# f90/Wave-U-Net

Measured on AMD Instinct MI355X. Metric: waveform samples/sec fwd+bwd, M1 12-level Wave-U-Net @1/2/4/8 GPU, higher is better.
Workload: dtype f32

## Files before the change

include/wun.h:

```cpp
#ifndef WUN_H
#define WUN_H

#include <stdint.h>

#ifdef __cplusplus
extern "C" {
#endif

typedef enum wun_status {
    WUN_OK = 0,
    WUN_ERR_INVALID = -1,
    WUN_ERR_UNSUPPORTED = -2,
    WUN_ERR_HIP = -3,
    WUN_ERR_NOMEM = -4
} wun_status;

typedef struct wun_config {
    int32_t num_layers;
    int32_t num_initial_filters;
    int32_t filter_size;
    int32_t merge_filter_size;
    int32_t input_filter_size;
    int32_t output_filter_size;
    int32_t upsampling;
// ... 512 lines not shown
#define WUN_OP_FIRST_CONV        7
#define WUN_PATH_NONE          0
#define WUN_PATH_SCALAR        1
#define WUN_PATH_VEC4          2
#define WUN_PATH_VEC8_BF16     3
#define WUN_PATH_ONE_STAGE     4
#define WUN_PATH_TWO_STAGE     5
#define WUN_PATH_GENERIC       6
#define WUN_PATH_FOUR_POSITION 7
#define WUN_PATH_NOT_FUSED     8
#define WUN_PATH_FUSED         9
#define WUN_PATH_FIRST_CONV    10
#define WUN_OP_WGRAD             8
#define WUN_PATH_WGRAD_DIRECT  11
#define WUN_PATH_WGRAD_SPLIT   12
int wun_op_last_path(int op);

int64_t wun_op_conv1d_bf16_scratch(int cin, int cout, int k);
int wun_op_conv1d_bf16(const float* x, const float* w, const float* bias, float* y, float* scratch,
                       int batch, int cin, int cout, int k, int t_in, int t_out, int stride, int pad_left,
                       int lrelu, void* stream);

int64_t wun_op_conv1d_dgrad_bf16_scratch(int cin, int cout, int k);
int wun_op_conv1d_dgrad_bf16(const float* dz, const float* w, float* dx, float* scratch, int batch, int cin,
                             int cout, int k, int t_in, int t_out, int stride, int pad_left, void* stream);

#define WUN_BF16_VARIANT_BASE 1000

typedef struct wun_op_conv_bf16_desc {
    int32_t mode, B, C0, C1, N, N0, K, Tin, Tout, shift;
// ... 48 lines not shown
```

wave-u-net_amd/_lib.py:

```python
import ctypes as C
import os

_HERE = os.path.dirname(os.path.abspath(__file__))
LIB_PATH = os.path.join(_HERE, os.environ.get("WUN_LIB", "libwun.so"))


class WunConfig(C.Structure):
    _fields_ = [(n, C.c_int32) for n in (
        "num_layers", "num_initial_filters", "filter_size", "merge_filter_size",
        "input_filter_size", "output_filter_size", "upsampling", "output_type", "context",
        "num_sources", "num_channels", "output_activation", "compute_dtype", "exclusive_streams")]


class WunPlanInfo(C.Structure):
    _fields_ = [("batch", C.c_int64), ("input_frames", C.c_int64), ("output_frames", C.c_int64),
                ("num_params", C.c_int64), ("arena_floats", C.c_int64),
                ("workspace_floats", C.c_int64), ("num_tensors", C.c_int64),
                ("num_outputs", C.c_int64), ("fwd_flops", C.c_double), ("bwd_flops", C.c_double),
                ("fwd_flops_dense", C.c_double), ("fwd_flops_unique", C.c_double),
                ("bwd_flops_unique", C.c_double), ("compute_dtype_effective", C.c_int64)]


class WunActivationInfo(C.Structure):
    _fields_ = [(n, C.c_int64) for n in ("offset", "batch_stride", "pitch", "channels", "frames", "t0", "tstep", "elem_bytes")]
# ... 58 lines not shown


class WunOpWgradDesc(C.Structure):
    _fields_ = ([(n, C.c_int32) for n in ("family", "B", "C0", "C1", "N", "K", "x0_pitch", "x1_pitch", "rows_bf16", "nparts")] +
                [(n, C.c_int32 * 2) for n in ("loader", "x0_off", "x1_off", "Tin", "shift", "Tq", "dz_pitch", "nsplit")] +
                [(n, C.c_int32) for n in ("accumulate", "force_mtw", "force_nw", "planes", "zss", "et")] +
                [("plane_off", C.c_int32 * 4)])


WGRAD_LDS, WGRAD_WIN, WGRAD_BF16, WGRAD_NARROW = range(4)
BF16_VARIANT_BASE = 1000

(OP_UPSAMPLE, OP_UPSAMPLE_BACKWARD, OP_INTERP_GRAD, OP_HEAD_FORWARD, OP_HEAD_DFEAT, OP_CONV_EPILOGUE, OP_BTC_TO_NCW) = range(7)
OP_FIRST_CONV = 7
OP_WGRAD = 8
(PATH_NONE, PATH_SCALAR, PATH_VEC4, PATH_VEC8_BF16, PATH_ONE_STAGE, PATH_TWO_STAGE, PATH_GENERIC, PATH_FOUR_POSITION,
 PATH_NOT_FUSED, PATH_FUSED, PATH_FIRST_CONV, PATH_WGRAD_DIRECT, PATH_WGRAD_SPLIT) = range(13)

BLEND_NO_RISE, BLEND_NO_FALL = 1, 2
SNIPPET_SWAP, SNIPPET_NEGATE = 1, 2
SPEED_RATES, SPEED_MAX_RATIO = 8, 64
STRETCH_JOBS = 64
SNIPPET_ROWS = 24

SPEC_TT_Z, SPEC_TT_MEAN, SPEC_TT_VAR, SPEC_TT_ACT, SPEC_TT_DROPOUT = range(5)

_P = C.c_void_p
_SIGS = {
    "wun_get_padding": (C.c_int, [C.POINTER(WunConfig), C.c_int64, C.POINTER(C.c_int64),
                                  C.POINTER(C.c_int64)]),
# ... 326 lines not shown
```

wave-u-net_amd/csrc/wun_internal.h:

```cpp
#pragma once
#include <hip/hip_runtime.h>
#include <stdint.h>
#include <initializer_list>
#include <string>

namespace wun {

enum { LOADER_DIRECT = 0, LOADER_DEINT = 1 };

enum WunEarlyWindow { EW_DEFAULT, EW_OFF, EW_DEEP, EW_ALL };
enum WunEventScope { EV_DEFAULT, EV_SYSTEM, EV_DEVICE };
enum WunSidePrio { PRIO_DEFAULT, PRIO_LOW, PRIO_HIGH, PRIO_NORMAL };
struct WunSwitches {
    bool no_dedup = false;
    WunEarlyWindow early_window = EW_DEFAULT;
    bool odd_fuse_set = false;
    int odd_fuse_min = 64;
    bool no_odd_align = false;
    bool no_fuse_ups = false;
    bool bf16_head_serial = false;
    bool single_stream = false;
    WunSidePrio side_prio = PRIO_DEFAULT;
    WunEventScope event_scope = EV_DEFAULT;
    bool no_win = false;
// ... 74 lines not shown
    int KW;
    int loader;
    const float* dz; long long dzbs; int dzpitch; int N; int Tq;
    float* out;
    int direct;
    int split_base;
    int nsplit; int units_per_split; int nQT; int B;
    int ablate;
    int force_mtw, force_nw;
    int bf16;
    int win;
    int sbf;
    int accum;
};

struct WgradGeom { int MTW, NW, nMG, nNG, TK, XP, ZP, nChMax, ONESP, XW4; size_t lds; };
WgradGeom wgrad_geom(const WgradArgs& a);
bool wgrad_win_supported(const WgradArgs& a);
long long wgrad_win_partial_floats(const WgradArgs& a, const WunSwitches& sw);
int wgrad_win_units(const WgradArgs& a, const WunSwitches& sw);
int wgrad_win_tiles(const WgradArgs& a, const WunSwitches& sw);
hipError_t launch_wgrad_win(const WgradArgs& a, hipStream_t s, const WunSwitches& sw);
hipError_t launch_wgrad_win_reduce(const WgradArgs& a, const float* partial, int nsplit, float* out_w, float* out_b,
                                   hipStream_t s, const WunSwitches& sw);
struct WgradBfGeom { int MTW, NW, NCB, nCB, nMG, nNG, TK, XW4, XROWS, ZPe; size_t lds; };
bool wgrad_bf16_supported(const WgradArgs& a);
WgradBfGeom wgrad_bf16_geom(const WgradArgs& a);
hipError_t launch_wgrad_bf16(const WgradArgs& a, hipStream_t s);
hipError_t launch_wgrad_bf16_reduce(const WgradArgs& a, const float* partial, int nsplit, float* out_w, float* out_b,
                                    hipStream_t s);

struct NarrowWgradArgs {
// ... 189 lines not shown
```

wave-u-net_amd/csrc/wun_kernels.hip:

```cpp
#include "wun_device.h"

#include <cstdio>
#include <cstdlib>
#include <map>
#include <mutex>
#include <string>
#include <algorithm>
#include <vector>

namespace wun {

__device__ __forceinline__ f32x4 mfma16(float a, float b, f32x4 c) {
    return __builtin_amdgcn_mfma_f32_16x16x4f32(a, b, c, 0, 0, 0);
}

__host__ __device__ static inline int fit_pitch(int width, int mod32) {
    return width + (((mod32 - (width % 32)) % 32) + 32) % 32;
}

struct ProfSlot { std::string name; std::string tag; double flops; double bytes; hipEvent_t e0, e1, c0, c1; };
static std::vector<ProfSlot> g_prof;
static bool g_prof_on = false;
static bool g_prof_detail = false;
static std::mutex g_prof_mu;
// ... 1234 lines not shown
        WUN_CV(24, 6, 2, 4, 1, 8) WUN_CV(25, 6, 3, 4, 1, 8)
        WUN_CV4(26, 4, 3, 4, 1, 4) WUN_CV4(27, 2, 3, 4, 1, 4) WUN_CV4(28, 3, 3, 4, 1, 4) WUN_CV4(29, 2, 2, 4, 1, 4)
        WUN_CV4(30, 3, 2, 4, 1, 4) WUN_CV4(31, 4, 5, 4, 1, 4) WUN_CV4(32, 3, 5, 4, 1, 4) WUN_CV4(33, 2, 5, 4, 1, 4)
#define WUN_CF(i, MT, NW, WT, WN, CK) case i: return conv_launch_t<MT, NW, WT, WN, CK, true, true>(a, v, part, part_cap, s, sw);
        WUN_CF(34, 1, 2, 4, 1, 8) WUN_CF(35, 1, 3, 4, 1, 8) WUN_CF(36, 2, 2, 4, 1, 8) WUN_CF(37, 2, 3, 4, 1, 8)
        WUN_CF(38, 2, 3, 2, 2, 8) WUN_CF(39, 4, 3, 2, 2, 8) WUN_CF(40, 2, 2, 2, 2, 8) WUN_CF(41, 4, 2, 2, 2, 8)
#undef WUN_CF
        default: return hipErrorInvalidValue;
    }
#undef WUN_CV
#undef WUN_CV4
}

#define WUN_WG_XIT 8

template <int MTW, int NW, bool ACC = false>
__global__ __launch_bounds__(256, 2) void wgrad_mfma_kernel(WgradArgs a, int nMG, int nNG, int TK,
                                                         int XP, int ZP, int nChMax, int ONESP,
                                                         int XW4) {
    extern __shared__ __attribute__((aligned(16))) float lds[];
    constexpr int MG = 4 * MTW * 16;
    constexpr int NG = NW * 16;
    constexpr int ZIT = (NG * 32 + 255) / 256;
    const bool deint = (a.loader == LOADER_DEINT);
    const int planes = deint ? 2 : 1;
    float* Xs = lds + ONESP;
    float* Zs = Xs + nChMax * planes * XP;

    const int tid = threadIdx.x;
    const int lane = tid & 63;
    const int li = lane & 15, lg = lane >> 4;
    const int wave = __builtin_amdgcn_readfirstlane(tid >> 6);
    int bid = xcd_contiguous_block((int)blockIdx.x, (int)gridDim.x);
    const int ng = bid % nNG; bid /= nNG;
    const int mg = bid % nMG;
    const int split = bid / nMG;

    const int Ctot = a.C0 + a.C1;
    const int Mtot = Ctot * a.KW;
    const int rlo = mg * MG;
    const int cLo = rlo / a.KW;
    int cHi = (rlo + MG - 1) / a.KW;
    if (cHi > Ctot - 1) cHi = Ctot - 1;
    const int nCh = cHi - cLo + 1;

    const int delta0 = ((a.off0 - a.shift) % 4 + 4) % 4;
    const int delta1 = ((a.off1 - a.shift) % 4 + 4) % 4;

    int rowoff[MTW];
    int nact = 0;
#pragma unroll
    for (int mt = 0; mt < MTW; ++mt) {
        const int rt = rlo + (wave * MTW + mt) * 16;
        if (rt <= Mtot) nact = mt + 1;
        const int r = rt + li;
        int off = 0;
        if (r < Mtot) {
            const int c = r / a.KW, k = r - c * a.KW;
            const int kd = k + (c < a.C0 ? delta0 : delta1);
            off = ONESP + (c - cLo) * planes * XP + (deint ? ((kd & 1) * XP + (kd >> 1)) : kd);
        }
        rowoff[mt] = off;
    }
    for (int i = tid; i < ONESP; i += 256) lds[i] = 1.f;

    f32x4 acc[MTW][NW];
#pragma unroll
    for (int m = 0; m < MTW; ++m)
#pragma unroll
        for (int n = 0; n < NW; ++n) acc[m][n] = (f32x4){0.f, 0.f, 0.f, 0.f};

    f32x4 xreg[WUN_WG_XIT];
    f32x4 zreg[ZIT];
    const int TK4 = TK >> 2;
    const float inv_xw4 = 1.0f / (float)XW4, inv_tk4 = 1.0f / (float)TK4;

    int xpk[WUN_WG_XIT];
    int zpk[ZIT];
#pragma unroll
    for (int i = 0; i < WUN_WG_XIT; ++i) {
        const int f = tid + i * 256;
        const int row = (int)(((float)f + 0.5f) * inv_xw4);
        const int c4 = f - row * XW4;
        const bool rok = row < nCh;
        const int ldsoff = deint ? (row * 2) * XP + 2 * c4 : row * XP + 4 * c4;
        xpk[i] = rok ? (int)(0x80000000u | ((unsigned)row << 23) | ((unsigned)c4 << 16) | (unsigned)ldsoff)
                     : (int)((unsigned)c4 << 16);
    }
#pragma unroll
    for (int i = 0; i < ZIT; ++i) {
        const int f = tid + i * 256;
        const int row = (int)(((float)f + 0.5f) * inv_tk4);
        const int c4 = f - row * TK4;
        zpk[i] = row < NG ? (int)(0x80000000u | ((unsigned)row << 23) | ((unsigned)c4 << 16) | (unsigned)(row * ZP + 4 * c4))
                          : (int)((unsigned)c4 << 16);
    }

    auto load_unit = [&](int u) {
        const int b = u / a.nQT, qt = u - b * a.nQT;
        const int q0 = qt * TK;
        const int tb = (deint ? 2 * q0 : q0) - a.shift;
        const float* base0 = a.src0 + (long long)b * a.bs0;
        const float* base1 = (a.C1 > 0) ? a.src1 + (long long)b * a.bs1 : base0;
        const int e00 = (tb + a.off0) & ~3, e01 = (tb + a.off1) & ~3;
#pragma unroll
        for (int i = 0; i < WUN_WG_XIT; ++i) {
            int pk = xpk[i];
            asm volatile("" : "+v"(pk));
            int c = cLo + ((pk >> 23) & 255);
            c = c < Ctot ? c : Ctot - 1;
            const bool s1 = c >= a.C0;
            const int xro = s1 ? (c - a.C0) * a.pitch1 : c * a.pitch0;
            int e = (s1 ? e01 : e00) + (((pk >> 16) & 127) << 2);
            const int emax = (s1 ? a.pitch1 : a.pitch0) - 4;
            e = e < 0 ? 0 : (e > emax ? emax : e);
            xreg[i] = *reinterpret_cast<const f32x4*>((s1 ? base1 : base0) + xro + e);
        }
        const float* zb = a.dz + (long long)b * a.dzbs;
        const int qmax = a.dzpitch - 4;
#pragma unroll
        for (int i = 0; i < ZIT; ++i) {
            int pk = zpk[i];
            asm volatile("" : "+v"(pk));
            const int nn = ng * NG + ((pk >> 23) & 255);
            const int zro = (pk < 0 && nn < a.N ? nn : 0) * a.dzpitch;
            int q = q0 + (((pk >> 16) & 127) << 2);
            q = q > qmax ? qmax : q;
            zreg[i] = *reinterpret_cast<const f32x4*>(zb + zro + q);
        }
    };
    auto store_unit = [&](int u) {
        const int b = u / a.nQT, qt = u - b * a.nQT;
        const int q0 = qt * TK;
        const int tb = (deint ? 2 * q0 : q0) - a.shift;
        int nq = a.Tq - q0; if (nq > TK) nq = TK;
        const int span = 4 * XW4;
        const int t00 = ((tb + a.off0) & ~3) - a.off0, t01 = ((tb + a.off1) & ~3) - a.off1;
        const bool xedge = t00 < 0 || t00 + span > a.Tin || (a.C1 > 0 && (t01 < 0 || t01 + span > a.Tin));
#pragma unroll
        for (int i = 0; i < WUN_WG_XIT; ++i) {
            int pk = xpk[i];
            asm volatile("" : "+v"(pk));
            if (pk < 0) {
                f32x4 v = xreg[i];
                if (xedge) {
                    const bool s1 = cLo + ((pk >> 23) & 255) >= a.C0;
                    const int t0 = (s1 ? t01 : t00) + (((pk >> 16) & 127) << 2);
#pragma unroll
                    for (int k = 0; k < 4; ++k)
                        if (t0 + k < 0 || t0 + k >= a.Tin) v[k] = 0.f;
                }
                float* dstp = Xs + (pk & 0xFFFF);
                if (!deint) {
                    *reinterpret_cast<f32x4*>(dstp) = v;
                } else {
                    *reinterpret_cast<float2*>(dstp) = make_float2(v[0], v[2]);
                    *reinterpret_cast<float2*>(dstp + XP) = make_float2(v[1], v[3]);
                }
            }
        }
        const bool zedge = nq < TK;
#pragma unroll
        for (int i = 0; i < ZIT; ++i) {
            int pk = zpk[i];
            asm volatile("" : "+v"(pk));
            if (pk < 0) {
                f32x4 v = zreg[i];
                if (zedge) {
                    const int c4x = ((pk >> 16) & 127) << 2;
#pragma unroll
                    for (int k = 0; k < 4; ++k)
                        if (c4x + k >= nq) v[k] = 0.f;
                }
                float* p = Zs + (pk & 0xFFFF);
                *reinterpret_cast<float2*>(p) = make_float2(v[0], v[1]);
                *reinterpret_cast<float2*>(p + 2) = make_float2(v[2], v[3]);
            }
        }
        (void)b;
    };

    const int nunits = a.B * a.nQT;
    const int u0 = split * a.units_per_split;
    int u1 = u0 + a.units_per_split;
    if (u1 > nunits) u1 = nunits;
    constexpr bool wb_noload = false, wb_nostore = false, wb_nomfma = false, wb_noepi = false;
    if (u0 < u1 && !wb_noload) load_unit(u0);
    for (int u = u0; u < u1; ++u) {
        const int qt = u % a.nQT;
        int nq = a.Tq - qt * TK; if (nq > TK) nq = TK;
        const int nsteps = (nq + 3) >> 2;
        __syncthreads();
        if (!wb_nostore) store_unit(u);
        __syncthreads();
        if (u + 1 < u1 && !wb_noload) load_unit(u + 1);
        if (!wb_nomfma) {
            auto run_unit = [&](auto full_tag) {
                constexpr bool FULL = decltype(full_tag)::value;
                float a0[MTW], b0[NW], a1[MTW], b1[NW];
                auto ldop = [&](int st, float (&av)[MTW], float (&bv)[NW]) {
#pragma unroll
                    for (int mt = 0; mt < MTW; ++mt) av[mt] = lds[rowoff[mt] + 4 * st + lg];
#pragma unroll
                    for (int n = 0; n < NW; ++n) bv[n] = Zs[(n * 16 + li) * ZP + 4 * st + lg];
                };
// ... 51 lines not shown
            for (int n = 0; n < NW; ++n) tile[(mt * NW + n) * 64] = acc[mt][n];
        return;
    }
    float* outp = a.out;
#pragma unroll
    for (int mt = 0; mt < MTW; ++mt) {
        if (mt >= nact) continue;
#pragma unroll
        for (int n = 0; n < NW; ++n) {
            const int col = ng * NG + n * 16 + li;
            if (col >= a.N) continue;
#pragma unroll
            for (int r4 = 0; r4 < 4; ++r4) {
                const int r = rlo + (wave * MTW + mt) * 16 + lg * 4 + r4;
                if (r < Mtot) {
                    const int c = r / a.KW, k = r - c * a.KW;
                    grad_st<ACC>(&outp[((long long)k * Ctot + c) * a.N + col], acc[mt][n][r4]);
                } else if (r == Mtot) {
                    grad_st<ACC>(&outp[(long long)Mtot * a.N + col], acc[mt][n][r4]);
                }
            }
        }
    }
}

struct WgradReduceArgs {
    const float* partial; float* out_w; float* out_b;
    int nsplit, MTW, NW, nMG, nNG, Mtot, KW, Ctot, N;
};

template <int SL, bool ACC = false>
// ... 17 lines not shown
            for (int j = 0; j < 8; ++j) t[j] = p[(long long)(k + j * SL) * sstride];
#pragma unroll
            for (int j = 0; j < 8; ++j) sum += t[j];
        }
        for (; k < a.nsplit; k += SL) sum += p[(long long)k * sstride];
    }
    if constexpr (SL > 1) {
        red[threadIdx.x] = sum;
        __syncthreads();
        if (sl != 0) return;
        sum = red[slot];
#pragma unroll
        for (int k = 1; k < SL; ++k) sum += red[k * VPB + slot];
    }
    if (!live) return;
    const int t = (int)(gv / tile_v), v = (int)(gv % tile_v);
    const int mg = t / a.nNG, ng = t % a.nNG;
    const int per_wave = a.MTW * a.NW * 64;
    const int wave = v / per_wave, rem = v % per_wave;
    const int tn = rem / 64, lane = rem % 64;
    const int mt = tn / a.NW, n = tn % a.NW;
    const int li = lane & 15, lg = lane >> 4;
    const int col = ng * NG + n * 16 + li;
    if (col >= a.N) return;
    const int r0 = mg * MG + (wave * a.MTW + mt) * 16 + lg * 4;
#pragma unroll
    for (int r4 = 0; r4 < 4; ++r4) {
        const int r = r0 + r4;
        if (r < a.Mtot) {
            const int c = r / a.KW, kk = r - c * a.KW;
            grad_st<ACC>(&a.out_w[((long long)kk * a.Ctot + c) * a.N + col], sum[r4]);
        } else if (r == a.Mtot) {
            grad_st<ACC>(&a.out_b[col], sum[r4]);
        }
    }
}


WgradGeom wgrad_geom(const WgradArgs& a) {
    WgradGeom g;
    const int Ctot = a.C0 + a.C1;
    const int mtiles = (Ctot * a.KW + 1 + 15) / 16;
    int bestnw = 3, bestpad = 1 << 30;
    for (int nw = 3; nw >= 1; --nw) {
        const int padded = ((a.N + nw * 16 - 1) / (nw * 16)) * nw * 16;
        if (padded < bestpad) { bestpad = padded; bestnw = nw; }
    }
    g.NW = (a.force_nw >= 1 && a.force_nw <= 5) ? a.force_nw : bestnw;
    int tk = (a.Tq + 3) & ~3;
    if (tk > 128) tk = 128;
    if (tk < 4) tk = 4;
    g.TK = tk;
    const bool deint = a.loader == LOADER_DEINT;
    const int Jx = deint ? (a.KW + 1) / 2 : a.KW;
    g.XW4 = deint ? (2 * (tk + Jx - 1) + 3 + 3) / 4 : (tk + a.KW - 1 + 3 + 3) / 4;
    const int mod = deint ? 10 : (a.KW >= 9 ? 16 : (a.KW >= 5 ? 8 : 4));
    g.XP = fit_pitch(deint ? 2 * g.XW4 : 4 * g.XW4, mod);
    g.ZP = fit_pitch(tk, 2);
    int mtw = mtiles <= 4 ? 1 : (mtiles <= 8 ? 2 : 6);
    if (a.force_mtw == 1 || a.force_mtw == 2 || a.force_mtw == 4 || a.force_mtw == 6) mtw = a.force_mtw;
    if (g.NW > 3 && mtw > 4) mtw = 4;
    g.ONESP = (tk + 15) & ~15;
    const int xit = WUN_WG_XIT;
    for (;;) {
        const int MG = 4 * mtw * 16;
        int nch = (MG + a.KW - 2) / a.KW + 1;
        if (nch > Ctot) nch = Ctot;
        g.nChMax = nch;
        if ((long long)nch * g.XW4 <= (long long)xit * 256 || mtw == 1) break;
        mtw = mtw == 6 ? 4 : (mtw == 4 ? 2 : 1);
    }
    g.MTW = mtw;
    const int MG = 4 * g.MTW * 16, NG = g.NW * 16;
    g.nMG = (Ctot * a.KW + 1 + MG - 1) / MG;
    g.nNG = (a.N + NG - 1) / NG;
    const size_t setb = (size_t)g.nChMax * (deint ? 2 : 1) * g.XP + (size_t)NG * g.ZP;
    g.lds = sizeof(float) * ((size_t)g.ONESP + setb);
    return g;
}

int wgrad_max_units(const WgradArgs& a, const WunSwitches& sw) {
    if (a.win) return wgrad_win_units(a, sw);
    const int TK = a.bf16 ? wgrad_bf16_geom(a).TK : wgrad_geom(a).TK;
    return a.B * ((a.Tq + TK - 1) / TK);
}

int wgrad_pick_nsplit(const WgradArgs& a, const WunSwitches& sw) {
    if (a.win) {
        const long long units = wgrad_win_units(a, sw), per = wgrad_win_tiles(a, sw);
        long long ns = (1024 + per - 1) / per;
        if (ns > units) ns = units;
        if (units >= 8 && ns > units / 2) ns = units / 2;
        if (ns < 1) ns = 1;
        const long long ups = (units + ns - 1) / ns;
        return (int)((units + ups - 1) / ups);
    }
    int TK, nMG, nNG;
    if (a.bf16) { const WgradBfGeom b = wgrad_bf16_geom(a); TK = b.TK; nMG = b.nMG; nNG = b.nNG; }
    else { const WgradGeom f = wgrad_geom(a); TK = f.TK; nMG = f.nMG; nNG = f.nNG; }
    const int nQT = (a.Tq + TK - 1) / TK;
    const long long units = (long long)a.B * nQT;
    const long long per = (long long)nMG * nNG;
    long long ns = (1024 + per - 1) / per;
    const long long blk = (long long)a.KW * (a.C0 + a.C1) * a.N;
    if (blk > (1ll << 18)) ns = (512 + per - 1) / per;
    if (ns > units) ns = units;
    if (ns < 1) ns = 1;
    if (units >= 8 && ns > units / 2) ns = units / 2;
    const long long ups = (units + ns - 1) / ns;
    ns = (units + ups - 1) / ups;
    return (int)ns;
}

template <int MTW, int NW>
static hipError_t wgrad_launch_t(WgradArgs a, const WgradGeom& g, hipStream_t s) {
    a.nQT = (a.Tq + g.TK - 1) / g.TK;
    const long long units = (long long)a.B * a.nQT;
    a.units_per_split = (int)((units + a.nsplit - 1) / a.nsplit);
    const bool acc = a.accum && a.direct;
    auto kern = acc ? wgrad_mfma_kernel<MTW, NW, true> : wgrad_mfma_kernel<MTW, NW>;
    static size_t lds_allowed[2] = {64 * 1024, 64 * 1024};
    size_t& allowed = lds_allowed[acc ? 1 : 0];
    if (g.lds > allowed) {
        hipError_t e = hipFuncSetAttribute((const void*)kern, hipFuncAttributeMaxDynamicSharedMemorySize, (int)g.lds);
        if (e != hipSuccess) return e;
        allowed = g.lds;
    }
    const long long grid = (long long)g.nMG * g.nNG * a.nsplit;
    char nm[64];
    snprintf(nm, sizeof(nm), acc ? "wgrad_mfma_acc_kernel<%d, %d>" : "wgrad_mfma_kernel<%d, %d>", MTW, NW);
    char tag[160];
    snprintf(tag, sizeof(tag), "C=%d N=%d T=%d K=%d ld=%d B=%d nsplit=%d grid=%lld", a.C0 + a.C1, a.N, a.Tq, a.KW,
             a.loader, a.B, a.nsplit, grid);
    ProfScope ps(nm, 2.0 * a.KW * (double)(a.C0 + a.C1) * a.N * (double)a.Tq * a.B, s, tag);
    hipLaunchKernelGGL(kern, dim3((unsigned)grid), dim3(256), g.lds, s, a, g.nMG, g.nNG, g.TK, g.XP,
                       g.ZP, g.nChMax, g.ONESP, g.XW4);
    return hipGetLastError();
}

hipError_t launch_wgrad(const WgradArgs& a, hipStream_t s, const WunSwitches& sw) {
    if (a.bf16) return launch_wgrad_bf16(a, s);
    if (a.win) return launch_wgrad_win(a, s, sw);
    if ((a.pitch0 & 3) || (a.bs0 & 3) || (reinterpret_cast<uintptr_t>(a.src0) & 15) || a.pitch0 < 4) return hipErrorInvalidValue;
    if (a.C1 > 0 && ((a.pitch1 & 3) || (a.bs1 & 3) || (reinterpret_cast<uintptr_t>(a.src1) & 15) || a.pitch1 < 4)) return hipErrorInvalidValue;
    if ((a.dzpitch & 3) || (a.dzbs & 3) || (reinterpret_cast<uintptr_t>(a.dz) & 15) || a.dzpitch < 4) return hipErrorInvalidValue;
    const WgradGeom g = wgrad_geom(a);
    if ((long long)g.nChMax * g.XW4 > (long long)WUN_WG_XIT * 256) return hipErrorInvalidValue;
#define WUN_WG(M, N) if (g.MTW == M && g.NW == N) return wgrad_launch_t<M, N>(a, g, s);
    WUN_WG(1, 1) WUN_WG(1, 2) WUN_WG(1, 3)
    WUN_WG(2, 1) WUN_WG(2, 2) WUN_WG(2, 3)
    WUN_WG(4, 1) WUN_WG(4, 2) WUN_WG(4, 3)
// ... 29 lines not shown
    if (a.bf16) { const WgradBfGeom b = wgrad_bf16_geom(a); return (long long)b.nMG * b.nNG * (4 * b.MTW * 16) * (b.NW * 16); }
    const WgradGeom g = wgrad_geom(a);
    return (long long)g.nMG * g.nNG * (4 * g.MTW * 16) * (g.NW * 16);
}

hipError_t launch_wgrad_reduce(const WgradArgs& a, const float* partial, int nsplit, float* out_w, float* out_b,
                               hipStream_t s, const WunSwitches& sw) {
    if (a.bf16) return launch_wgrad_bf16_reduce(a, partial, nsplit, out_w, out_b, s);
    if (a.win) return launch_wgrad_win_reduce(a, partial, nsplit, out_w, out_b, s, sw);
    const WgradGeom g = wgrad_geom(a);
    WgradReduceArgs r;
    r.partial = partial; r.out_w = out_w; r.out_b = out_b;
    r.nsplit = nsplit; r.MTW = g.MTW; r.NW = g.NW; r.nMG = g.nMG; r.nNG = g.nNG;
    r.Ctot = a.C0 + a.C1; r.KW = a.KW; r.Mtot = r.Ctot * a.KW; r.N = a.N;
    const long long slots = (long long)g.nMG * g.nNG * (4 * g.MTW * 16) * (g.NW * 16) / 4;
    const int sl = (nsplit >= 64 && slots < (1 << 16)) ? 16 : (nsplit >= 8 && slots < (1 << 18) ? 4 : 1);
    const int vpb = 256 / sl;
    const long long blocks = (slots + vpb - 1) / vpb;
    char tag[96];
    snprintf(tag, sizeof(tag), "bytes=%lld nsplit=%d", (long long)((nsplit + 1) * slots * 16), nsplit);
    ProfScope ps(a.accum ? "wgrad_reduce_acc_kernel" : "wgrad_reduce_kernel", 0.0, s, tag, (double)((nsplit + 1) * slots * 16));
    if (a.accum) {
        if (sl == 16) hipLaunchKernelGGL((wgrad_reduce_kernel<16, true>), dim3((unsigned)blocks), dim3(256), 0, s, r);
        else if (sl == 4) hipLaunchKernelGGL((wgrad_reduce_kernel<4, true>), dim3((unsigned)blocks), dim3(256), 0, s, r);
        else hipLaunchKernelGGL((wgrad_reduce_kernel<1, true>), dim3((unsigned)blocks), dim3(256), 0, s, r);
        return hipGetLastError();
    }
    if (sl == 16) hipLaunchKernelGGL(wgrad_reduce_kernel<16>, dim3((unsigned)blocks), dim3(256), 0, s, r);
    else if (sl == 4) hipLaunchKernelGGL(wgrad_reduce_kernel<4>, dim3((unsigned)blocks), dim3(256), 0, s, r);
    else hipLaunchKernelGGL(wgrad_reduce_kernel<1>, dim3((unsigned)blocks), dim3(256), 0, s, r);
// ... 20 lines not shown
```

wave-u-net_amd/csrc/wun_op.hip:

```cpp
#include "wun_plan_impl.h"

#include <algorithm>
#include <cstdio>
#include <cstdlib>
#include <cstring>

namespace wun {
hipError_t launch_make_wt_one(const float* src, float* dst, WtDesc d, hipStream_t s);
}

static const long long kOpScratchFloats = 8ll << 20;
static int g_op_variant = -1, g_op_ksplit = 0;
static int g_op_wg_mtw = 0, g_op_wg_nw = 0, g_op_wg_nsplit = 0;
static int g_op_wg_bf16 = 0;
static int g_op_wg_narrow = 0;
static int g_op_wg_win = 0;
static float* g_op_copy0 = nullptr; static float* g_op_copy1 = nullptr;
static int g_op_copy_t0 = 0, g_op_copy_t1 = 0, g_op_copy_exp = 0, g_op_copy_lo = 0, g_op_copy_len = 0, g_op_acc_lo = 0, g_op_acc_len = 0;
static float* g_op_ups_y = nullptr; static const float* g_op_ups_w = nullptr;
static int g_op_ups_pitch = 0, g_op_ups_tup = 0;
static thread_local int t_op_epilogue_path = WUN_PATH_NONE;
static thread_local int t_op_first_conv_path = WUN_PATH_NONE;
static thread_local int t_op_wgrad_path = WUN_PATH_NONE, t_op_wgrad_splits = 0;
static float* op_scratch() {
    static float* buf = nullptr;
    if (!buf && hipMalloc((void**)&buf, kOpScratchFloats * sizeof(float)) != hipSuccess) {
        buf = nullptr;
        (void)hipGetLastError();
    }
    return buf;
}

static void* op_bf16_tmp(int slot, size_t bytes) {
    static void* buf[2] = {nullptr, nullptr};
    static size_t cap[2] = {0, 0};
    if (bytes > cap[slot]) {
        (void)hipDeviceSynchronize();
// ... 419 lines not shown
    HIP_TRY(launch_btc_to_ncw(src, dst, B, T, C, pitch, (hipStream_t)stream));
    return WUN_OK;
}

extern "C" int wun_op_last_path(int op) {
    switch (op) {
        case WUN_OP_UPSAMPLE: return elementwise_last_path(EW_UPSAMPLE);
        case WUN_OP_UPSAMPLE_BACKWARD: return elementwise_last_path(EW_UPSAMPLE_BWD);
        case WUN_OP_INTERP_GRAD: return elementwise_last_path(EW_INTERP_GRAD);
        case WUN_OP_HEAD_FORWARD: return elementwise_last_path(EW_HEAD_FWD);
        case WUN_OP_HEAD_DFEAT: return elementwise_last_path(EW_HEAD_DFEAT);
        case WUN_OP_BTC_TO_NCW: return elementwise_last_path(EW_BTC_TO_NCW);
        case WUN_OP_CONV_EPILOGUE: return t_op_epilogue_path;
        case WUN_OP_FIRST_CONV: return t_op_first_conv_path;
        case WUN_OP_WGRAD: return t_op_wgrad_path;
        default: return fail(WUN_ERR_INVALID, "unknown operator");
    }
}
static_assert(EW_PATH_SCALAR == WUN_PATH_SCALAR && EW_PATH_VEC4 == WUN_PATH_VEC4 && EW_PATH_VEC8_BF16 == WUN_PATH_VEC8_BF16 &&
              EW_PATH_ONE_STAGE == WUN_PATH_ONE_STAGE && EW_PATH_TWO_STAGE == WUN_PATH_TWO_STAGE &&
              EW_PATH_GENERIC == WUN_PATH_GENERIC && EW_PATH_FOUR_POSITION == WUN_PATH_FOUR_POSITION, "wun.h path values");

extern "C" int wun_op_set_conv_copies(float* copy0, int t0, int expand, int exp_lo, int exp_len, float* copy1, int t1,
                                      int acc_lo, int acc_len) {
    if ((copy0 && t0 < 1) || (copy1 && t1 < 1) || exp_len < 0 || acc_len < 0) return fail(WUN_ERR_INVALID, "bad copy geometry");
    g_op_copy0 = copy0; g_op_copy_t0 = t0; g_op_copy_exp = expand ? 1 : 0; g_op_copy_lo = exp_lo; g_op_copy_len = exp_len;
    g_op_copy1 = copy1; g_op_copy_t1 = t1; g_op_acc_lo = acc_lo; g_op_acc_len = acc_len;
    return WUN_OK;
}

extern "C" int64_t wun_op_conv1d_bf16_scratch(int cin, int cout, int k) {
// ... 319 lines not shown
extern "C" int64_t wun_op_wgrad_ex_scratch(const wun_op_wgrad_desc* d) {
    OpWgrad o;
    if (int rc = op_wgrad_build(d, nullptr, nullptr, nullptr, nullptr, wun_switches_from_env(), o)) return rc;
    return (int64_t)o.total * o.part_floats + 128;
}

extern "C" int wun_op_wgrad_max_units(const wun_op_wgrad_desc* d, int part) {
    OpWgrad o;
    if (int rc = op_wgrad_build(d, nullptr, nullptr, nullptr, nullptr, wun_switches_from_env(), o)) return rc;
    if (part < 0 || part >= o.nparts) return fail(WUN_ERR_INVALID, "no such part");
    return o.units[part];
}

extern "C" int wun_op_wgrad_last_splits(void) { return t_op_wgrad_splits; }

extern "C" int wun_op_wgrad_ex(const wun_op_wgrad_desc* d, const void* x0, const void* x1, const void* dz_part0,
                               const void* dz_part1, float* grads, float* scratch, void* stream) {
    if (!d || !x0 || !dz_part0 || !grads || !scratch || (d->C1 > 0 && !x1) || (d->nparts == 2 && !dz_part1))
        return fail(WUN_ERR_INVALID, "null argument");
    if (reinterpret_cast<uintptr_t>(grads) & 3) return fail(WUN_ERR_INVALID, "grads not aligned to a float");
    const WunSwitches sw = wun_switches_from_env();
    OpWgrad o;
    if (int rc = op_wgrad_build(d, x0, x1, dz_part0, dz_part1, sw, o)) return rc;
    hipStream_t s = (hipStream_t)stream;
    float* partial = (float*)(((uintptr_t)scratch + 255) & ~(uintptr_t)255);
    if (o.narrow) {
        int done = 0;
        for (int i = 0; i < o.nparts; ++i) {
            o.nw[i].partial = partial; o.nw[i].split_base = done;
            HIP_TRY(launch_narrow_wgrad(o.nw[i], s, sw));
            done += o.nw[i].nsplit;
        }
        HIP_TRY(launch_narrow_wgrad_reduce(o.nw[0], partial, o.total, grads, o.woff, o.boff, s, d->accumulate != 0));
        t_op_wgrad_path = WUN_PATH_WGRAD_SPLIT; t_op_wgrad_splits = o.total;
        return WUN_OK;
    }
    float* out_w = grads;
    float* out_b = out_w + (long long)d->K * (d->C0 + d->C1) * d->N;
    if (o.total == 1) {
        o.w[0].out = out_w; o.w[0].direct = 1; o.w[0].split_base = 0;
// ... 27 lines not shown
```

Before: 33.04 million.

## Fold several short batch items into one wgrad MFMA time tile

```diff
diff --git a/include/wun.h b/include/wun.h
--- a/include/wun.h
+++ b/include/wun.h
@@ -550,6 +550,7 @@
 #define WUN_OP_WGRAD             8
 #define WUN_PATH_WGRAD_DIRECT  11
 #define WUN_PATH_WGRAD_SPLIT   12
+#define WUN_OP_WGRAD_UNITS       9
 int wun_op_last_path(int op);
 
 int64_t wun_op_conv1d_bf16_scratch(int cin, int cout, int k);
diff --git a/wave-u-net_amd/_lib.py b/wave-u-net_amd/_lib.py
--- a/wave-u-net_amd/_lib.py
+++ b/wave-u-net_amd/_lib.py
@@ -96,6 +96,7 @@
 (OP_UPSAMPLE, OP_UPSAMPLE_BACKWARD, OP_INTERP_GRAD, OP_HEAD_FORWARD, OP_HEAD_DFEAT, OP_CONV_EPILOGUE, OP_BTC_TO_NCW) = range(7)
 OP_FIRST_CONV = 7
 OP_WGRAD = 8
+OP_WGRAD_UNITS = 9
 (PATH_NONE, PATH_SCALAR, PATH_VEC4, PATH_VEC8_BF16, PATH_ONE_STAGE, PATH_TWO_STAGE, PATH_GENERIC, PATH_FOUR_POSITION,
  PATH_NOT_FUSED, PATH_FUSED, PATH_FIRST_CONV, PATH_WGRAD_DIRECT, PATH_WGRAD_SPLIT) = range(13)
 
diff --git a/wave-u-net_amd/csrc/wun_internal.h b/wave-u-net_amd/csrc/wun_internal.h
--- a/wave-u-net_amd/csrc/wun_internal.h
+++ b/wave-u-net_amd/csrc/wun_internal.h
@@ -112,8 +112,9 @@
     int accum;
 };
 
-struct WgradGeom { int MTW, NW, nMG, nNG, TK, XP, ZP, nChMax, ONESP, XW4; size_t lds; };
+struct WgradGeom { int MTW, NW, nMG, nNG, TK, XP, ZP, nChMax, ONESP, XW4, nQT, FOLD, SEG; size_t lds; };
 WgradGeom wgrad_geom(const WgradArgs& a);
+static inline int wgrad_geom_units(const WgradGeom& g, int B) { return ((B + g.FOLD - 1) / g.FOLD) * g.nQT; }
 bool wgrad_win_supported(const WgradArgs& a);
 long long wgrad_win_partial_floats(const WgradArgs& a, const WunSwitches& sw);
 int wgrad_win_units(const WgradArgs& a, const WunSwitches& sw);
diff --git a/wave-u-net_amd/csrc/wun_kernels.hip b/wave-u-net_amd/csrc/wun_kernels.hip
--- a/wave-u-net_amd/csrc/wun_kernels.hip
+++ b/wave-u-net_amd/csrc/wun_kernels.hip
@@ -1272,10 +1272,10 @@
 
 #define WUN_WG_XIT 8
 
-template <int MTW, int NW, bool ACC = false>
+template <int MTW, int NW, bool ACC = false, bool FOLDED = false>
 __global__ __launch_bounds__(256, 2) void wgrad_mfma_kernel(WgradArgs a, int nMG, int nNG, int TK,
                                                          int XP, int ZP, int nChMax, int ONESP,
-                                                         int XW4) {
+                                                         int XW4, int FOLD, int SEG) {
     extern __shared__ __attribute__((aligned(16))) float lds[];
     constexpr int MG = 4 * MTW * 16;
     constexpr int NG = NW * 16;
@@ -1297,8 +1297,9 @@
     const int Ctot = a.C0 + a.C1;
     const int Mtot = Ctot * a.KW;
     const int rlo = mg * MG;
-    const int cLo = rlo / a.KW;
-    int cHi = (rlo + MG - 1) / a.KW;
+    const float inv_kw = 1.0f / (float)a.KW;
+    const int cLo = fast_div(rlo, a.KW, inv_kw);
+    int cHi = fast_div(rlo + MG - 1, a.KW, inv_kw);
     if (cHi > Ctot - 1) cHi = Ctot - 1;
     const int nCh = cHi - cLo + 1;
 
@@ -1314,7 +1315,7 @@
         const int r = rt + li;
         int off = 0;
         if (r < Mtot) {
-            const int c = r / a.KW, k = r - c * a.KW;
+            const int c = fast_div(r, a.KW, inv_kw), k = r - c * a.KW;
             const int kd = k + (c < a.C0 ? delta0 : delta1);
             off = ONESP + (c - cLo) * planes * XP + (deint ? ((kd & 1) * XP + (kd >> 1)) : kd);
         }
@@ -1332,6 +1333,8 @@
     f32x4 zreg[ZIT];
     const int TK4 = TK >> 2;
     const float inv_xw4 = 1.0f / (float)XW4, inv_tk4 = 1.0f / (float)TK4;
+    constexpr bool fold = FOLDED;
+    const float inv_seg = 1.0f / (float)SEG, inv_nqt = 1.0f / (float)a.nQT;
 
     int xpk[WUN_WG_XIT];
     int zpk[ZIT];
@@ -1354,13 +1357,26 @@
                           : (int)((unsigned)c4 << 16);
     }
 
+    auto unit_origin = [&](int u, int& b0, int& q0) {
+        if constexpr (FOLDED) { b0 = u * FOLD; q0 = 0; return; }
+        const int ub = fast_div(u, a.nQT, inv_nqt);
+        b0 = ub;
+        q0 = (u - ub * a.nQT) * TK;
+    };
+    auto seg_of = [&](int p, int es, float inv_es, int& g, int& o) {
+        if constexpr (FOLDED) { g = fast_div(p, es, inv_es); o = p - g * es; }
+        else { g = 0; o = p; }
+    };
+    const int ES = planes * SEG;
+    const float inv_es = 1.0f / (float)ES;
+
     auto load_unit = [&](int u) {
-        const int b = u / a.nQT, qt = u - b * a.nQT;
-        const int q0 = qt * TK;
+        int b0, q0;
+        unit_origin(u, b0, q0);
         const int tb = (deint ? 2 * q0 : q0) - a.shift;
-        const float* base0 = a.src0 + (long long)b * a.bs0;
-        const float* base1 = (a.C1 > 0) ? a.src1 + (long long)b * a.bs1 : base0;
         const int e00 = (tb + a.off0) & ~3, e01 = (tb + a.off1) & ~3;
+        const float* base0 = a.src0 + (long long)b0 * a.bs0;
+        const float* base1 = (a.C1 > 0) ? a.src1 + (long long)b0 * a.bs1 : base0;
 #pragma unroll
         for (int i = 0; i < WUN_WG_XIT; ++i) {
             int pk = xpk[i];
@@ -1369,12 +1385,20 @@
             c = c < Ctot ? c : Ctot - 1;
             const bool s1 = c >= a.C0;
             const int xro = s1 ? (c - a.C0) * a.pitch1 : c * a.pitch0;
-            int e = (s1 ? e01 : e00) + (((pk >> 16) & 127) << 2);
+            int g, o;
+            seg_of(((pk >> 16) & 127) << 2, ES, inv_es, g, o);
+            int e = (s1 ? e01 : e00) + o;
             const int emax = (s1 ? a.pitch1 : a.pitch0) - 4;
             e = e < 0 ? 0 : (e > emax ? emax : e);
-            xreg[i] = *reinterpret_cast<const f32x4*>((s1 ? base1 : base0) + xro + e);
-        }
-        const float* zb = a.dz + (long long)b * a.dzbs;
+            const float* base = s1 ? base1 : base0;
+            if constexpr (FOLDED) {
+                int b = b0 + g;
+                b = b < a.B ? b : a.B - 1;
+                base = s1 ? a.src1 + (long long)b * a.bs1 : a.src0 + (long long)b * a.bs0;
+            }
+            xreg[i] = *reinterpret_cast<const f32x4*>(base + xro + e);
+        }
+        const float* zb = a.dz + (long long)b0 * a.dzbs;
         const int qmax = a.dzpitch - 4;
 #pragma unroll
         for (int i = 0; i < ZIT; ++i) {
@@ -1382,19 +1406,27 @@
             asm volatile("" : "+v"(pk));
             const int nn = ng * NG + ((pk >> 23) & 255);
             const int zro = (pk < 0 && nn < a.N ? nn : 0) * a.dzpitch;
-            int q = q0 + (((pk >> 16) & 127) << 2);
+            int g, o;
+            seg_of(((pk >> 16) & 127) << 2, SEG, inv_seg, g, o);
+            int q = q0 + o;
             q = q > qmax ? qmax : q;
-            zreg[i] = *reinterpret_cast<const f32x4*>(zb + zro + q);
+            const float* zp = zb;
+            if constexpr (FOLDED) {
+                int b = b0 + g;
+                b = b < a.B ? b : a.B - 1;
+                zp = a.dz + (long long)b * a.dzbs;
+            }
+            zreg[i] = *reinterpret_cast<const f32x4*>(zp + zro + q);
         }
     };
     auto store_unit = [&](int u) {
-        const int b = u / a.nQT, qt = u - b * a.nQT;
-        const int q0 = qt * TK;
+        int b0, q0;
+        unit_origin(u, b0, q0);
         const int tb = (deint ? 2 * q0 : q0) - a.shift;
         int nq = a.Tq - q0; if (nq > TK) nq = TK;
         const int span = 4 * XW4;
         const int t00 = ((tb + a.off0) & ~3) - a.off0, t01 = ((tb + a.off1) & ~3) - a.off1;
-        const bool xedge = t00 < 0 || t00 + span > a.Tin || (a.C1 > 0 && (t01 < 0 || t01 + span > a.Tin));
+        const bool xedge = fold || t00 < 0 || t00 + span > a.Tin || (a.C1 > 0 && (t01 < 0 || t01 + span > a.Tin));
 #pragma unroll
         for (int i = 0; i < WUN_WG_XIT; ++i) {
             int pk = xpk[i];
@@ -1403,10 +1435,13 @@
                 f32x4 v = xreg[i];
                 if (xedge) {
                     const bool s1 = cLo + ((pk >> 23) & 255) >= a.C0;
-                    const int t0 = (s1 ? t01 : t00) + (((pk >> 16) & 127) << 2);
+                    int g, o;
+                    seg_of(((pk >> 16) & 127) << 2, ES, inv_es, g, o);
+                    const int t0 = (s1 ? t01 : t00) + o;
+                    const bool dead = FOLDED && b0 + g >= a.B;
 #pragma unroll
                     for (int k = 0; k < 4; ++k)
-                        if (t0 + k < 0 || t0 + k >= a.Tin) v[k] = 0.f;
+                        if (dead || t0 + k < 0 || t0 + k >= a.Tin) v[k] = 0.f;
                 }
                 float* dstp = Xs + (pk & 0xFFFF);
                 if (!deint) {
@@ -1417,7 +1452,7 @@
                 }
             }
         }
-        const bool zedge = nq < TK;
+        const bool zedge = fold || nq < TK;
 #pragma unroll
         for (int i = 0; i < ZIT; ++i) {
             int pk = zpk[i];
@@ -1425,28 +1460,34 @@
             if (pk < 0) {
                 f32x4 v = zreg[i];
                 if (zedge) {
-                    const int c4x = ((pk >> 16) & 127) << 2;
+                    int g, o;
+                    seg_of(((pk >> 16) & 127) << 2, SEG, inv_seg, g, o);
+                    const int lim = (!FOLDED || b0 + g < a.B) ? a.Tq - q0 : 0;
 #pragma unroll
                     for (int k = 0; k < 4; ++k)
-                        if (c4x + k >= nq) v[k] = 0.f;
+                        if (o + k >= lim) v[k] = 0.f;
                 }
                 float* p = Zs + (pk & 0xFFFF);
                 *reinterpret_cast<float2*>(p) = make_float2(v[0], v[1]);
                 *reinterpret_cast<float2*>(p + 2) = make_float2(v[2], v[3]);
             }
         }
-        (void)b;
     };
 
-    const int nunits = a.B * a.nQT;
+    const int nunits = FOLDED ? (a.B + FOLD - 1) / FOLD : a.B * a.nQT;
     const int u0 = split * a.units_per_split;
     int u1 = u0 + a.units_per_split;
     if (u1 > nunits) u1 = nunits;
     constexpr bool wb_noload = false, wb_nostore = false, wb_nomfma = false, wb_noepi = false;
     if (u0 < u1 && !wb_noload) load_unit(u0);
     for (int u = u0; u < u1; ++u) {
-        const int qt = u % a.nQT;
-        int nq = a.Tq - qt * TK; if (nq > TK) nq = TK;
+        int b0, q0;
+        unit_origin(u, b0, q0);
+        int nq = a.Tq - q0; if (nq > TK) nq = TK;
+        if (fold) {
+            int nseg = a.B - b0; if (nseg > FOLD) nseg = FOLD;
+            nq = (nseg - 1) * SEG + a.Tq;
+        }
         const int nsteps = (nq + 3) >> 2;
         __syncthreads();
         if (!wb_nostore) store_unit(u);
@@ -1528,7 +1569,7 @@
             for (int r4 = 0; r4 < 4; ++r4) {
                 const int r = rlo + (wave * MTW + mt) * 16 + lg * 4 + r4;
                 if (r < Mtot) {
-                    const int c = r / a.KW, k = r - c * a.KW;
+                    const int c = fast_div(r, a.KW, inv_kw), k = r - c * a.KW;
                     grad_st<ACC>(&outp[((long long)k * Ctot + c) * a.N + col], acc[mt][n][r4]);
                 } else if (r == Mtot) {
                     grad_st<ACC>(&outp[(long long)Mtot * a.N + col], acc[mt][n][r4]);
@@ -1576,12 +1617,14 @@
         for (int k = 1; k < SL; ++k) sum += red[k * VPB + slot];
     }
     if (!live) return;
-    const int t = (int)(gv / tile_v), v = (int)(gv % tile_v);
-    const int mg = t / a.nNG, ng = t % a.nNG;
+    const unsigned gb = blockIdx.x * (unsigned)VPB;
+    const int t = (int)(gb / (unsigned)tile_v), v = (int)(gb - (unsigned)t * (unsigned)tile_v) + slot;
+    const int mg = t / a.nNG, ng = t - mg * a.nNG;
     const int per_wave = a.MTW * a.NW * 64;
-    const int wave = v / per_wave, rem = v % per_wave;
-    const int tn = rem / 64, lane = rem % 64;
-    const int mt = tn / a.NW, n = tn % a.NW;
+    const int wave = fast_div(v, per_wave, 1.0f / (float)per_wave), rem = v - wave * per_wave;
+    const int tn = rem >> 6, lane = rem & 63;
+    const int mt = fast_div(tn, a.NW, 1.0f / (float)a.NW), n = tn - mt * a.NW;
+    const float inv_kw = 1.0f / (float)a.KW;
     const int li = lane & 15, lg = lane >> 4;
     const int col = ng * NG + n * 16 + li;
     if (col >= a.N) return;
@@ -1590,7 +1633,7 @@
     for (int r4 = 0; r4 < 4; ++r4) {
         const int r = r0 + r4;
         if (r < a.Mtot) {
-            const int c = r / a.KW, kk = r - c * a.KW;
+            const int c = fast_div(r, a.KW, inv_kw), kk = r - c * a.KW;
             grad_st<ACC>(&a.out_w[((long long)kk * a.Ctot + c) * a.N + col], sum[r4]);
         } else if (r == a.Mtot) {
             grad_st<ACC>(&a.out_b[col], sum[r4]);
@@ -1599,7 +1642,7 @@
 }
 
 
-WgradGeom wgrad_geom(const WgradArgs& a) {
+static WgradGeom wgrad_geom_for(const WgradArgs& a, int tk, int nqt, int fold, int seg) {
     WgradGeom g;
     const int Ctot = a.C0 + a.C1;
     const int mtiles = (Ctot * a.KW + 1 + 15) / 16;
@@ -1609,10 +1652,7 @@
         if (padded < bestpad) { bestpad = padded; bestnw = nw; }
     }
     g.NW = (a.force_nw >= 1 && a.force_nw <= 5) ? a.force_nw : bestnw;
-    int tk = (a.Tq + 3) & ~3;
-    if (tk > 128) tk = 128;
-    if (tk < 4) tk = 4;
-    g.TK = tk;
+    g.TK = tk; g.nQT = nqt; g.FOLD = fold; g.SEG = seg;
     const bool deint = a.loader == LOADER_DEINT;
     const int Jx = deint ? (a.KW + 1) / 2 : a.KW;
     g.XW4 = deint ? (2 * (tk + Jx - 1) + 3 + 3) / 4 : (tk + a.KW - 1 + 3 + 3) / 4;
@@ -1641,9 +1681,39 @@
     return g;
 }
 
+static long long wgrad_unit_cost(const WgradGeom& g, long long ksteps, long long units) {
+    return (long long)g.nMG * g.nNG * (ksteps * 64 * g.MTW * g.NW + units * 1500);
+}
+
+WgradGeom wgrad_geom(const WgradArgs& a) {
+    const int nqt = a.Tq > 128 ? (a.Tq + 127) / 128 : 1;
+    int tk = ((a.Tq + nqt - 1) / nqt + 3) & ~3;
+    if (tk < 4) tk = 4;
+    const int unfolded_seg = 1 << 16;
+    const WgradGeom g = wgrad_geom_for(a, tk, nqt, 1, unfolded_seg);
+    if (nqt > 1 || a.B < 2) return g;
+    const bool deint = a.loader == LOADER_DEINT;
+    const int reach = deint ? (a.KW + 2) >> 1 : a.KW + 2;
+    const int seg = (a.Tq + reach + 3) & ~3;
+    int fold = 128 / seg;
+    if (fold > a.B) fold = a.B;
+    WgradGeom f = g;
+    for (; fold >= 3; --fold) {
+        f = wgrad_geom_for(a, fold * seg, 1, fold, seg);
+        if (f.MTW == g.MTW && (long long)f.nChMax * f.XW4 <= (long long)WUN_WG_XIT * 256) break;
+    }
+    if (fold < 3) return g;
+    const long long full = a.B / fold, rest = a.B - full * fold;
+    long long fsteps = full * (((fold - 1) * seg + a.Tq + 3) >> 2);
+    if (rest > 0) fsteps += ((rest - 1) * seg + a.Tq + 3) >> 2;
+    const long long gsteps = (long long)a.B * ((a.Tq + 3) >> 2);
+    return wgrad_unit_cost(f, fsteps, full + (rest > 0)) < wgrad_unit_cost(g, gsteps, a.B) ? f : g;
+}
+
 int wgrad_max_units(const WgradArgs& a, const WunSwitches& sw) {
     if (a.win) return wgrad_win_units(a, sw);
-    const int TK = a.bf16 ? wgrad_bf16_geom(a).TK : wgrad_geom(a).TK;
+    if (!a.bf16) return wgrad_geom_units(wgrad_geom(a), a.B);
+    const int TK = wgrad_bf16_geom(a).TK;
     return a.B * ((a.Tq + TK - 1) / TK);
 }
 
@@ -1657,11 +1727,10 @@
         const long long ups = (units + ns - 1) / ns;
         return (int)((units + ups - 1) / ups);
     }
-    int TK, nMG, nNG;
-    if (a.bf16) { const WgradBfGeom b = wgrad_bf16_geom(a); TK = b.TK; nMG = b.nMG; nNG = b.nNG; }
-    else { const WgradGeom f = wgrad_geom(a); TK = f.TK; nMG = f.nMG; nNG = f.nNG; }
-    const int nQT = (a.Tq + TK - 1) / TK;
-    const long long units = (long long)a.B * nQT;
+    int nMG, nNG;
+    long long units;
+    if (a.bf16) { const WgradBfGeom b = wgrad_bf16_geom(a); nMG = b.nMG; nNG = b.nNG; units = (long long)a.B * ((a.Tq + b.TK - 1) / b.TK); }
+    else { const WgradGeom f = wgrad_geom(a); nMG = f.nMG; nNG = f.nNG; units = wgrad_geom_units(f, a.B); }
     const long long per = (long long)nMG * nNG;
     long long ns = (1024 + per - 1) / per;
     const long long blk = (long long)a.KW * (a.C0 + a.C1) * a.N;
@@ -1676,13 +1745,15 @@
 
 template <int MTW, int NW>
 static hipError_t wgrad_launch_t(WgradArgs a, const WgradGeom& g, hipStream_t s) {
-    a.nQT = (a.Tq + g.TK - 1) / g.TK;
-    const long long units = (long long)a.B * a.nQT;
+    a.nQT = g.nQT;
+    const long long units = wgrad_geom_units(g, a.B);
     a.units_per_split = (int)((units + a.nsplit - 1) / a.nsplit);
     const bool acc = a.accum && a.direct;
-    auto kern = acc ? wgrad_mfma_kernel<MTW, NW, true> : wgrad_mfma_kernel<MTW, NW>;
-    static size_t lds_allowed[2] = {64 * 1024, 64 * 1024};
-    size_t& allowed = lds_allowed[acc ? 1 : 0];
+    const bool folded = g.FOLD > 1;
+    auto kern = folded ? (acc ? wgrad_mfma_kernel<MTW, NW, true, true> : wgrad_mfma_kernel<MTW, NW, false, true>)
+                       : (acc ? wgrad_mfma_kernel<MTW, NW, true> : wgrad_mfma_kernel<MTW, NW>);
+    static size_t lds_allowed[4] = {64 * 1024, 64 * 1024, 64 * 1024, 64 * 1024};
+    size_t& allowed = lds_allowed[(acc ? 1 : 0) + (folded ? 2 : 0)];
     if (g.lds > allowed) {
         hipError_t e = hipFuncSetAttribute((const void*)kern, hipFuncAttributeMaxDynamicSharedMemorySize, (int)g.lds);
         if (e != hipSuccess) return e;
@@ -1692,11 +1763,11 @@
     char nm[64];
     snprintf(nm, sizeof(nm), acc ? "wgrad_mfma_acc_kernel<%d, %d>" : "wgrad_mfma_kernel<%d, %d>", MTW, NW);
     char tag[160];
-    snprintf(tag, sizeof(tag), "C=%d N=%d T=%d K=%d ld=%d B=%d nsplit=%d grid=%lld", a.C0 + a.C1, a.N, a.Tq, a.KW,
-             a.loader, a.B, a.nsplit, grid);
+    snprintf(tag, sizeof(tag), "C=%d N=%d T=%d K=%d ld=%d B=%d nsplit=%d grid=%lld TK=%d fold=%d units=%lld", a.C0 + a.C1, a.N, a.Tq, a.KW,
+             a.loader, a.B, a.nsplit, grid, g.TK, g.FOLD, units);
     ProfScope ps(nm, 2.0 * a.KW * (double)(a.C0 + a.C1) * a.N * (double)a.Tq * a.B, s, tag);
     hipLaunchKernelGGL(kern, dim3((unsigned)grid), dim3(256), g.lds, s, a, g.nMG, g.nNG, g.TK, g.XP,
-                       g.ZP, g.nChMax, g.ONESP, g.XW4);
+                       g.ZP, g.nChMax, g.ONESP, g.XW4, g.FOLD, g.SEG);
     return hipGetLastError();
 }
 
@@ -1756,6 +1827,7 @@
     r.nsplit = nsplit; r.MTW = g.MTW; r.NW = g.NW; r.nMG = g.nMG; r.nNG = g.nNG;
     r.Ctot = a.C0 + a.C1; r.KW = a.KW; r.Mtot = r.Ctot * a.KW; r.N = a.N;
     const long long slots = (long long)g.nMG * g.nNG * (4 * g.MTW * 16) * (g.NW * 16) / 4;
+    if (slots >= (1ll << 31)) return hipErrorInvalidValue;
     const int sl = (nsplit >= 64 && slots < (1 << 16)) ? 16 : (nsplit >= 8 && slots < (1 << 18) ? 4 : 1);
     const int vpb = 256 / sl;
     const long long blocks = (slots + vpb - 1) / vpb;
diff --git a/wave-u-net_amd/csrc/wun_op.hip b/wave-u-net_amd/csrc/wun_op.hip
--- a/wave-u-net_amd/csrc/wun_op.hip
+++ b/wave-u-net_amd/csrc/wun_op.hip
@@ -21,6 +21,7 @@
 static int g_op_ups_pitch = 0, g_op_ups_tup = 0;
 static thread_local int t_op_epilogue_path = WUN_PATH_NONE;
 static thread_local int t_op_first_conv_path = WUN_PATH_NONE;
+static thread_local int t_op_wgrad_unit[2][4] = {{0, 0, 0, 0}, {0, 0, 0, 0}};
 static thread_local int t_op_wgrad_path = WUN_PATH_NONE, t_op_wgrad_splits = 0;
 static float* op_scratch() {
     static float* buf = nullptr;
@@ -470,7 +471,9 @@
         case WUN_OP_CONV_EPILOGUE: return t_op_epilogue_path;
         case WUN_OP_FIRST_CONV: return t_op_first_conv_path;
         case WUN_OP_WGRAD: return t_op_wgrad_path;
-        default: return fail(WUN_ERR_INVALID, "unknown operator");
+        default:
+            if (op >= WUN_OP_WGRAD_UNITS && op < WUN_OP_WGRAD_UNITS + 8) return t_op_wgrad_unit[(op - WUN_OP_WGRAD_UNITS) >> 2][(op - WUN_OP_WGRAD_UNITS) & 3];
+            return fail(WUN_ERR_INVALID, "unknown operator");
     }
 }
 static_assert(EW_PATH_SCALAR == WUN_PATH_SCALAR && EW_PATH_VEC4 == WUN_PATH_VEC4 && EW_PATH_VEC8_BF16 == WUN_PATH_VEC8_BF16 &&
@@ -820,6 +823,16 @@
 
 extern "C" int wun_op_wgrad_last_splits(void) { return t_op_wgrad_splits; }
 
+static void op_wgrad_note_units(const OpWgrad& o, int family) {
+    memset(t_op_wgrad_unit, 0, sizeof(t_op_wgrad_unit));
+    if (family != WUN_WGRAD_LDS) return;
+    for (int i = 0; i < o.nparts; ++i) {
+        const WgradGeom g = wgrad_geom(o.w[i]);
+        t_op_wgrad_unit[i][0] = g.TK; t_op_wgrad_unit[i][1] = g.nQT; t_op_wgrad_unit[i][2] = g.FOLD;
+        t_op_wgrad_unit[i][3] = g.FOLD > 1 ? g.SEG : 0;
+    }
+}
+
 extern "C" int wun_op_wgrad_ex(const wun_op_wgrad_desc* d, const void* x0, const void* x1, const void* dz_part0,
                                const void* dz_part1, float* grads, float* scratch, void* stream) {
     if (!d || !x0 || !dz_part0 || !grads || !scratch || (d->C1 > 0 && !x1) || (d->nparts == 2 && !dz_part1))
@@ -830,6 +843,7 @@
     if (int rc = op_wgrad_build(d, x0, x1, dz_part0, dz_part1, sw, o)) return rc;
     hipStream_t s = (hipStream_t)stream;
     float* partial = (float*)(((uintptr_t)scratch + 255) & ~(uintptr_t)255);
+    op_wgrad_note_units(o, d->family);
     if (o.narrow) {
         int done = 0;
         for (int i = 0; i < o.nparts; ++i) {
```

After: 33.02 million (median of 4 runs). About the same (-0.1%).
